# Yelp/nrtsearch

Hardware: AMD Instinct MI355X
Metric: queries/sec, 10M-doc 5-term BM25 top-1000 (higher is better)
Workload: dtype f32

## Files before the change

nrtsearch_amd/csrc/maxscore.hip:

```cpp
#include <hip/hip_runtime.h>
#include <stdint.h>

#include <type_traits>

#include "bm25_common.hiph"

namespace nrtgpu {

constexpr int kMsWinWords = kMsWinDocs / 32;
constexpr int kSl = kMsSlots;
typedef uint32_t u32x2 __attribute__((ext_vector_type(2)));
typedef const NRT_GLOBAL u32x2* gvec2_ptr;

struct alignas(16) WClause {
  uint64_t docids, fnorm;
  uint64_t begin;
  uint32_t count, pad0;
  float    weight;
  int32_t  fx_scale;
  uint32_t flags;
  uint32_t pad;
  uint64_t u_after;
  uint64_t look;
  uint64_t cells, start;
};
static_assert(sizeof(WClause) == 80, "WClause layout");

struct MsSmem {
  uint64_t cand[kMsCandCap];
  uint32_t tab[kTabTerms][kTabEntries];
  float    cache[kLdsCaches][256];
  uint32_t seen[kMsWaves][kMsWinWords];
  WClause  wc[kMsWaves][kMsMaxTerms];
  TopkScratch sc;
  uint64_t theta;
  uint64_t thr;
  uint32_t cnt;
  uint32_t cnt_valid;
  uint32_t rz_flag;
  uint32_t spec_busy;
  uint32_t spec_meet;
  uint32_t n_meet, n_over, n_est;
  uint32_t wins_started;
  uint32_t spec_at;
  uint32_t q_wins;
  uint32_t spec_z16;
  uint32_t spec_grow16;
  unsigned long long* spec_slot;
  uint64_t pick;
  uint32_t role[4];
  uint32_t prune_on;
  uint32_t slot_hits[kSliceSlots];
  uint32_t slot_slice[kSliceSlots];
  uint64_t prof[16];
};
static_assert(sizeof(MsSmem) <= 160 * 1024, "the MaxScore workgroup owns one CU's 160 KiB LDS");

__device__ __forceinline__ uint64_t uniform_u64(uint64_t v) {
  const uint32_t lo = (uint32_t)__builtin_amdgcn_readfirstlane((int)(uint32_t)v);
  const uint32_t hi = (uint32_t)__builtin_amdgcn_readfirstlane((int)(uint32_t)(v >> 32));
  return ((uint64_t)hi << 32) | (uint64_t)lo;
}
__device__ __forceinline__ uint64_t readlane_u64(uint64_t v, uint32_t l) {
  const uint32_t lo = (uint32_t)__builtin_amdgcn_readlane((int)(uint32_t)v, (int)l);
  const uint32_t hi = (uint32_t)__builtin_amdgcn_readlane((int)(uint32_t)(v >> 32), (int)l);
  return ((uint64_t)hi << 32) | (uint64_t)lo;
}

template <bool PACKED, int NS>
__device__ __forceinline__ void values_of_codes(const MsSmem& s, const uint32_t (&c)[NS], uint32_t need, uint32_t tab_slot,
                                                float w, int fx_scale, uint32_t cache_slot, uint64_t esc_list,
                                                const uint32_t (&pidx)[NS], uint32_t (&val)[NS]) {
  const uint32_t tab = tab_slot < (uint32_t)kTabTerms ? tab_slot : 7u;
  const char* tb = (const char*)&s.tab[tab == 7u ? 0u : tab][0];
  uint32_t cor = 0;
#pragma unroll
  for (int j = 0; j < NS; ++j) {
    val[j] = *(const uint32_t*)(tb + (c[j] & 0x1FFCu));
    const uint32_t cn = ((need >> j) & 1u) ? c[j] : 0u;
    cor = PACKED ? max(cor, cn) : (cor | cn);
  }
  const bool special = need != 0u && ((PACKED ? cor >= (kPackEscBase << 2) : (cor >> 31) != 0u) || tab == 7u);
  if (__any(special)) {
    const float* cache = &s.cache[cache_slot][0];
#pragma unroll
    for (int j = 0; j < NS; ++j) {
      uint32_t cj = c[j];
      if (PACKED && cj >= (kPackEscBase << 2)) cj = ((need >> j) & 1u) ? packed_escape_word((gu32_ptr)esc_list, pidx[j], cj >> 2) : 0x80000100u;
      const bool esc = (cj >> 31) != 0u;
      const uint32_t f = esc ? ((cj >> 8) & 0x3FFFFFu) : ((cj >> 9) & 15u);
      const bool dead = esc ? ((cj >> 30) & 1u) != 0u : (cj >> 20) != 0u;
      const uint32_t nb = esc ? (cj & 255u) : ((cj >> 2) & 127u);
      if (((need >> j) & 1u) && (esc || tab == 7u))
        val[j] = dead ? 0u : score_value<true>(bm25_score(w, (float)(int32_t)f, cache[nb]), fx_scale);
    }
  }
}

#ifdef NRT_MS_PHASE_CLOCKS
#define NRT_PH_MARK(i)                                                          \
  do {                                                                          \
    if (PROF) {                                                                 \
      asm volatile("s_waitcnt vmcnt(0) lgkmcnt(0)" ::: "memory");               \
      const uint64_t t_ph_ = __builtin_readcyclecounter();                      \
      ph[i] += t_ph_ - ph_t;                                                    \
      ph_t = t_ph_;                                                             \
    }                                                                           \
  } while (0)
#else
#define NRT_PH_MARK(i) do {} while (0)
#endif
typedef const __attribute__((address_space(4))) MsArgs* ms_args_ptr;
template <class T>
__device__ __forceinline__ T* as_global(T* p) { return (T*)(NRT_GLOBAL T*)p; }
__device__ __forceinline__ ms_args_ptr ms_fresh(const MsArgs* p) {
  uint32_t lo = (uint32_t)(uintptr_t)p, hi = (uint32_t)((uintptr_t)p >> 32);
  asm volatile("" : "+v"(lo), "+v"(hi));
  lo = (uint32_t)__builtin_amdgcn_readfirstlane((int)lo);
  hi = (uint32_t)__builtin_amdgcn_readfirstlane((int)hi);
  return (ms_args_ptr)(((uintptr_t)hi << 32) | (uintptr_t)lo);
}

__device__ __noinline__ void ms_compact(__attribute__((address_space(3))) MsSmem* sp, uint32_t k, int fx_E,
                                        unsigned long long* theta_g, const DExchange* xch, uint32_t query) {
  MsSmem& s = *(MsSmem*)sp;
  const uint32_t tid = threadIdx.x;
  const uint32_t cnt_raw = s.cnt;
  const uint32_t cnt0 = cnt_raw > (uint32_t)kMsCandCap ? s.cnt_valid : cnt_raw;
#ifdef NRTGPU_DEV
  const bool keep_live = (s.spec_meet & 4u) == 0u;
#else
  constexpr bool keep_live = true;
#endif
  const uint64_t tg_in = tid == 0 && keep_live ? (uint64_t)__hip_atomic_load(theta_g, __ATOMIC_RELAXED, __HIP_MEMORY_SCOPE_AGENT) : 0ull;
  __syncthreads();
  if (tid == 0) {
    s.n_meet += 1u;
    if (cnt_raw > (uint32_t)kMsCandCap) s.n_over += 1u;
    if (tg_in > s.theta) {
      s.theta = tg_in;
      s.thr = acc_threshold<true>(tg_in, fx_E);
    }
  }
  const bool exchanging = xch && xch->world > 1u;
  uint32_t r = 0;
  if (s.spec_z16 != 0u && !exchanging && __hip_atomic_load(&s.prune_on, __ATOMIC_RELAXED, __HIP_MEMORY_SCOPE_WORKGROUP) != 0u) {
    const float m = (float)k * fminf(1.0f, (float)s.wins_started / (float)max(s.q_wins, 1u));
    const float rr = m + (float)s.spec_z16 * (1.0f / 16.0f) * sqrtf(m) + 2.0f;
    r = rr < (float)k ? (uint32_t)rr : 0u;
  }
  uint64_t guess = 0;
  if (cnt0 > k) {
    const uint32_t k2 = exchanging ? (k + xch->world - 2u) / (xch->world - 1u) : r;
    const uint64_t thr = topk_kth_union<kMsThreads>(s.cand, cnt0, k, &s.sc, [](auto&&) {}, k2);
    const uint32_t q2_hi = s.sc.q2_hi;
    uint64_t keep = thr;
    if (keep_live) {
      const uint64_t edge = !exchanging && r != 0u && q2_hi != 0u ? (uint64_t)q2_hi << 32 : 0ull, th_in = s.theta;
      if (edge > keep) keep = edge;
      if (th_in > keep) keep = th_in;
    }
    const uint32_t kept = topk_keep_ge<kMsThreads, kMsCandCap>(s.cand, cnt0, keep, &s.sc);
    for (uint32_t i = kept + tid; i < (uint32_t)kMsCandCap; i += kMsThreads) s.cand[i] = 0ull;
    if (tid == 0) {
      s.cnt = kept;
      if (thr > s.theta) {
        s.theta = thr;
        s.thr = acc_threshold<true>(thr, fx_E);
      }
      atomicMax(theta_g, (unsigned long long)thr);
      s.prof[1] += 1;
    }
    if (!exchanging && r != 0u && q2_hi != 0u) guess = (uint64_t)q2_hi << 32;
    if (xch && tid < 64u) {
      const uint64_t pb = exchange_bound(*xch, query, q2_hi != 0u ? (uint64_t)q2_hi << 32 : 0ull, tid);
      if (tid == 0 && pb > s.theta) {
        s.theta = pb;
        s.thr = acc_threshold<true>(pb, fx_E);
        atomicMax(theta_g, (unsigned long long)pb);
      }
    }
  } else {
    if (r != 0u && cnt0 > r) guess = topk_kth_union<kMsThreads>(s.cand, cnt0, r, &s.sc, [](auto&&) {}, 0u);
    if (tid == 0) s.cnt = cnt0;
  }
  if (tid == 0 && s.spec_z16 != 0u) {
    if (guess > s.theta) {
      s.theta = guess;
      s.thr = acc_threshold<true>(guess, fx_E);
      atomicMax(theta_g, (unsigned long long)guess);
      atomicMax(s.spec_slot, (unsigned long long)guess);
      s.n_est += 0x10000u;
    }
    const uint32_t ws = s.wins_started;
    s.spec_at = ws >= s.q_wins ? 0u : max(ws * s.spec_grow16 / 16u, ws + (uint32_t)kMsWaves);
  }
  __syncthreads();
  if (tid == 0) s.rz_flag = 0;
  __syncthreads();
}

__device__ __forceinline__ bool ms_meet(MsSmem& s, uint32_t k, int fx_E, unsigned long long* theta_g, const DExchange* xch = nullptr,
                                        uint32_t query = 0) {
  __syncthreads();
  if (!__hip_atomic_load(&s.rz_flag, __ATOMIC_RELAXED, __HIP_MEMORY_SCOPE_WORKGROUP)) return false;
  ms_compact((__attribute__((address_space(3))) MsSmem*)&s, k, fx_E, theta_g, xch, query);
  return true;
}

__device__ __noinline__ void ms_estimate(__attribute__((address_space(3))) MsSmem* sp, uint32_t k, int fx_E,
                                         unsigned long long* theta_g, const DExchange* xch) {
  MsSmem& s = *(MsSmem*)sp;
  const uint32_t lane = threadIdx.x & 63u;
  const uint32_t ws = (uint32_t)__builtin_amdgcn_readfirstlane((int)__hip_atomic_load(&s.wins_started, __ATOMIC_RELAXED, __HIP_MEMORY_SCOPE_WORKGROUP));
  const uint32_t at = (uint32_t)__builtin_amdgcn_readfirstlane((int)__hip_atomic_load(&s.spec_at, __ATOMIC_RELAXED, __HIP_MEMORY_SCOPE_WORKGROUP));
  const uint32_t n = (uint32_t)__builtin_amdgcn_readfirstlane((int)__hip_atomic_load(&s.cnt, __ATOMIC_RELAXED, __HIP_MEMORY_SCOPE_WORKGROUP));
  if (at != 0u && ws >= at && n <= (uint32_t)kMsCandCap) {
    const bool exchanging = xch && xch->world > 1u;
    uint32_t r = 0;
    if (s.spec_z16 != 0u && !exchanging && __hip_atomic_load(&s.prune_on, __ATOMIC_RELAXED, __HIP_MEMORY_SCOPE_WORKGROUP) != 0u) {
      const float m = (float)k * fminf(1.0f, (float)ws / (float)max(s.q_wins, 1u));
      const float rr = m + (float)s.spec_z16 * (1.0f / 16.0f) * sqrtf(m) + 2.0f;
      r = rr < (float)k ? (uint32_t)rr : 0u;
    }
    uint64_t guess = 0;
    if (r != 0u && n > r) guess = topk_kth_wave(s.cand, n, r, &s.sc);
    if (lane == 0u) {
      if (guess > s.theta) {
        __hip_atomic_store(&s.theta, guess, __ATOMIC_RELAXED, __HIP_MEMORY_SCOPE_WORKGROUP);
        __hip_atomic_store(&s.thr, acc_threshold<true>(guess, fx_E), __ATOMIC_RELAXED, __HIP_MEMORY_SCOPE_WORKGROUP);
        atomicMax(theta_g, (unsigned long long)guess);
        atomicMax(s.spec_slot, (unsigned long long)guess);
      }
      s.spec_at = ws >= s.q_wins ? 0u : max(ws * s.spec_grow16 / 16u, ws + (uint32_t)kMsWaves);
      s.n_est += 1u;
    }
  }
  wave_lds_phase();
  if (lane == 0u) __hip_atomic_store(&s.spec_busy, 0u, __ATOMIC_RELEASE, __HIP_MEMORY_SCOPE_WORKGROUP);
}

__device__ __forceinline__ bool ms_reserve(MsSmem& s, uint32_t lane, uint32_t mine, uint32_t& pos) {
  const uint32_t incl = scan64_dpp(mine);
  const uint32_t wave_total = (uint32_t)__builtin_amdgcn_readlane((int)incl, 63);
  uint32_t wbase = 0;
  if (lane == 0) {
    wbase = atomicAdd(&s.cnt, wave_total);
    if (wbase + wave_total > (uint32_t)kMsCandCap) {
      if (wbase <= (uint32_t)kMsCandCap) s.cnt_valid = wbase;
      __hip_atomic_store(&s.rz_flag, 1u, __ATOMIC_RELAXED, __HIP_MEMORY_SCOPE_WORKGROUP);
    }
  }
  wbase = (uint32_t)__builtin_amdgcn_readfirstlane((int)wbase);
  pos = wbase + incl - mine;
  return wbase + wave_total <= (uint32_t)kMsCandCap;
}

template <bool PROF, bool PACKED, int SHAPES>
__global__ __launch_bounds__(kMsThreads)
void bm25_maxscore_kernel(const MsArgs* __restrict__ launch) {
  constexpr bool TWO = SHAPES == 2;
  constexpr bool kMsHalfBody = kSl == 8;
  __shared__ MsSmem s;
  const uint32_t tid = threadIdx.x;
  const uint32_t wave = tid >> 6, lane = tid & 63u;
  for (uint32_t round = 0;; ++round) {
    const uint64_t wall_entry = PROF ? wall_clock64() : 0ull;
    const ms_args_ptr ap = ms_fresh(launch);
    const __attribute__((address_space(4))) DHelp& hp = ap->help;
    const DItem* const items = as_global(ap->items);
    const DPart* const parts = as_global(ap->parts);
    const DWalkRow* const rows = as_global(ap->rows);
  #ifdef NRTGPU_DEV
    const DTerm* const terms = as_global(ap->terms);
  #endif
    const DExchange* const xch = as_global(ap->xch);
    bool helper = false;
    uint32_t my_item = 0, out_slot = 0;
    {
      const uint32_t min_rem = hp.min_rem & 0xFFFFu;
      const bool greedy = ((hp.min_rem >> 16) & 1u) != 0u;
      for (int attempt = 0; attempt < 2; ++attempt) {
        if (tid == 0) {
          s.pick = 0ull;
          s.role[0] = __hip_atomic_load(hp.item_next, __ATOMIC_RELAXED, __HIP_MEMORY_SCOPE_AGENT);
          s.role[1] = __hip_atomic_load(hp.help_used, __ATOMIC_RELAXED, __HIP_MEMORY_SCOPE_AGENT);
          s.role[2] = 0u;
          s.role[3] = __hip_atomic_load(hp.help_off, __ATOMIC_RELAXED, __HIP_MEMORY_SCOPE_AGENT);
        }
        __syncthreads();
        const uint32_t q_next = s.role[0];
        const bool queue_empty = attempt == 1 || q_next >= hp.n_own;
        const bool slots_left = s.role[1] < hp.n_help;
        if (queue_empty && (!slots_left || s.role[3] != 0u)) return;
        const bool look = slots_left && (queue_empty || (hp.alpha16 != 0u && q_next >= hp.n_cus + hp.n_cus / 4u));
        if (look) {
          const uint64_t now = wall_clock64();
          float t_rem = 0.f;
          if (!queue_empty) {
            uint32_t mine = 0;
            for (uint32_t i = tid; i < hp.n_own; i += kMsThreads) {
              const uint64_t t0 = __hip_atomic_load(hp.item_t0 + i, __ATOMIC_RELAXED, __HIP_MEMORY_SCOPE_AGENT);
              if (t0 == 0ull) continue;
              mine += min(items[i].flags >> 8, (uint32_t)kMsWaves + __hip_atomic_load(hp.win_next + i, __ATOMIC_RELAXED, __HIP_MEMORY_SCOPE_AGENT));
            }
            mine = (uint32_t)__builtin_amdgcn_readlane((int)scan64_dpp(mine), 63);
            if (lane == 0 && mine != 0u) atomicAdd(&s.role[2], mine);
            __syncthreads();
            const uint32_t handed = s.role[2];
            const uint64_t ts = __hip_atomic_load(hp.t_start, __ATOMIC_RELAXED, __HIP_MEMORY_SCOPE_AGENT);
            t_rem = (handed == 0u || ts == 0ull || now <= ts) ? 3.0e38f
                    : (float)(now - ts) * (float)(hp.total_wins > handed ? hp.total_wins - handed : 0u) / (float)handed * ((float)hp.alpha16 * (1.0f / 16.0f));
          }
          for (uint32_t i = tid; i < hp.n_own; i += kMsThreads) {
            const uint32_t fl = items[i].flags;
            if ((fl & 3u) == kMsModeExact) continue;
            const uint32_t nw = fl >> 8;
            const uint32_t taken = (uint32_t)kMsWaves + __hip_atomic_load(hp.win_next + i, __ATOMIC_RELAXED, __HIP_MEMORY_SCOPE_AGENT);
            if (taken + min_rem > nw) continue;
            const uint64_t t0 = __hip_atomic_load(hp.item_t0 + i, __ATOMIC_RELAXED, __HIP_MEMORY_SCOPE_AGENT);
            if (t0 == 0ull || now <= t0) continue;
            const uint32_t hc = __hip_atomic_load(hp.help_cnt + i, __ATOMIC_RELAXED, __HIP_MEMORY_SCOPE_AGENT);
            const float left = (float)(now - t0) * (float)(nw - taken) / ((float)(taken - (uint32_t)kMsWaves + 1u) * (float)(1u + hc));
            if (!queue_empty && !(left > t_rem)) continue;
            uint32_t hsh = ((blockIdx.x + round * gridDim.x) * 0x9E3779B9u) ^ (i * 0x85EBCA6Bu) ^ (uint32_t)now;
            hsh ^= hsh >> 16; hsh *= 0x7FEB352Du; hsh ^= hsh >> 15; hsh *= 0x846CA68Bu; hsh ^= hsh >> 16;
            const float u = ((float)(hsh >> 8) + 0.5f) * (1.0f / 16777216.0f);
            const float key = greedy ? left : left / -__logf(u);
            atomicMax((unsigned long long*)&s.pick, ((unsigned long long)__float_as_uint(key) << 32) | (unsigned long long)(i + 1u));
          }
        }
        __syncthreads();
        if (tid == 0) {
          const uint64_t pick = s.pick;
          uint32_t r_item = 0xFFFFFFFFu, r_slot = 0xFFFFFFFFu;
          if ((uint32_t)pick != 0u) {
            const uint32_t slot = atomicAdd(hp.help_used, 1u);
            if (slot < hp.n_help) {
              r_slot = slot;
              r_item = (uint32_t)pick - 1u;
              atomicAdd(hp.help_cnt + r_item, 1u);
            }
          } else if (queue_empty && look) {
            __hip_atomic_store(hp.help_off, 1u, __ATOMIC_RELAXED, __HIP_MEMORY_SCOPE_AGENT);
          }
          if (r_slot == 0xFFFFFFFFu && !queue_empty) {
            const uint32_t it = atomicAdd(hp.item_next, 1u);
            if (it < hp.n_own) r_item = it;
          }
          s.role[0] = r_item;
          s.role[1] = r_slot;
        }
        __syncthreads();
        const uint32_t r_item = s.role[0], r_slot = s.role[1];
        __syncthreads();
        if (r_item != 0xFFFFFFFFu) {
          my_item = r_item;
          helper = r_slot != 0xFFFFFFFFu;
          out_slot = helper ? hp.slot_base + r_slot : r_item;
          break;
        }
        if (queue_empty) return;
      }
    }
    NRT_GLOBAL uint32_t* const win_next_g = (NRT_GLOBAL uint32_t*)(hp.win_next + my_item);
    uint32_t first_win = 0;
    if (helper && lane == 0) first_win = __hip_atomic_fetch_add(win_next_g, 1u, __ATOMIC_RELAXED, __HIP_MEMORY_SCOPE_AGENT);
    const DItem item = items[my_item];
    const DQuery q = as_global(ap->queries)[item.query];
    const uint32_t k = q.k;
    const int fx_E = item.fx_E;
    unsigned long long* const my_theta_g = as_global(ap->theta_g) + item.query;
    const bool multi_item = q.n_items > 1 || hp.n_help != 0u;
    const uint32_t mode = item.flags & 3u;
    const uint32_t win_tiles = (uint32_t)kMsWinTiles >> ((item.flags >> 2) & 3u);
    const uint32_t msm = SHAPES ? q.min_should_match : 0u;
    const bool use_max = SHAPES && q.combine_max != 0u;
    const uint32_t sec_mode = TWO ? q.sec_mode : kMsSecNone;
    const float tie_breaker = TWO ? q.tie_breaker : 0.0f;
    auto loosen = [&](uint64_t t) { return (TWO && sec_mode == kMsSecReqOpt) ? max(t - (t >> 21), (uint64_t)2) - (uint64_t)1 : t; };
    unsigned int* const my_prune_g = as_global(ap->q_prune) + item.query;
    const uint64_t after_key = q.has_after ? pack_key(q.after_score, (uint32_t)q.after_doc) : ~0ull;

    {
      const uint32_t n_lds = min(item.n_caches, (uint32_t)kLdsCaches) * 256u;
      const float* const caches = as_global(ap->caches);
      for (uint32_t i = tid; i < n_lds; i += kMsThreads) (&s.cache[0][0])[i] = caches[item.cache_off + i];
    }
    for (uint32_t i = tid; i < (uint32_t)kMsCandCap; i += kMsThreads) s.cand[i] = 0ull;
    if (tid == 0) {
      const uint64_t theta0 = __hip_atomic_load(my_theta_g, __ATOMIC_RELAXED, __HIP_MEMORY_SCOPE_AGENT);
      s.theta = theta0;
      s.thr = acc_threshold<true>(theta0, fx_E);
      s.cnt = 0;
      s.cnt_valid = 0;
      s.rz_flag = 0;
      s.spec_busy = 0;
      s.n_meet = s.n_over = s.n_est = 0;
      if (!helper) {
        const unsigned long long now0 = (unsigned long long)wall_clock64();
        __hip_atomic_store(hp.item_t0 + my_item, now0, __ATOMIC_RELAXED, __HIP_MEMORY_SCOPE_AGENT);
        if (my_item == 0u) __hip_atomic_store(hp.t_start, now0, __ATOMIC_RELAXED, __HIP_MEMORY_SCOPE_AGENT);
      }
      s.prune_on = mode == kMsModePrune ? 1u : 0u;
      const bool spec = hp.spec_g != nullptr && hp.spec_z16 != 0u;
      s.wins_started = 0;
      s.q_wins = spec ? as_global(ap->q_wins)[item.query] : 0u;
      s.spec_z16 = spec ? hp.spec_z16 : 0u;
      s.spec_slot = spec ? as_global(hp.spec_g) + item.query : nullptr;
      s.spec_at = spec ? max(hp.spec_sched & 255u, 1u) : 0u;
      s.spec_grow16 = max((hp.spec_sched >> 8) & 255u, 17u);
      s.spec_meet = (hp.spec_sched >> 16) & 7u;
      for (int i = 0; i < kSliceSlots; ++i) s.slot_hits[i] = s.slot_slice[i] = 0u;
      for (int i = 0; i < 16; ++i) s.prof[i] = 0;
    }
    const uint64_t t_item0 = PROF ? __builtin_readcyclecounter() : 0ull;
    const uint64_t wall0 = PROF ? wall_clock64() : 0ull;
    uint64_t tc_meet = 0, tc_part = 0, tc_walk = 0;
    __syncthreads();
    if (xch && tid < 64u) {
      const uint64_t pb = exchange_bound(*xch, item.query, 0ull, tid);
      if (tid == 0 && pb > s.theta) {
        s.theta = pb;
        s.thr = acc_threshold<true>(pb, fx_E);
      }
    }
    for (uint32_t slot = 0; slot < item.n_tabs; ++slot) {
      const float w = items[my_item].tab_weight[slot];
      const int scale = items[my_item].tab_scale[slot];
      const float* cache = &s.cache[items[my_item].tab_cache[slot]][0];
      for (uint32_t e = tid; e < (uint32_t)kTabEntries; e += kMsThreads)
        s.tab[slot][e] = e < (uint32_t)kTabNorms ? 0u : score_value<true>(bm25_score(w, (float)(int32_t)(e >> 7), cache[e & 127u]), scale);
    }
    __syncthreads();
  #if !defined(NRT_MS_PHASE_CLOCKS) && !defined(NRT_MS_COUNT_ROUNDS)
    if (PROF && tid == 0) s.prof[8] = __builtin_readcyclecounter() - t_item0;
  #endif

    uint32_t* const seen = &s.seen[wave][0];
    WClause* const wcl = &s.wc[wave][0];
    const uint32_t wcl_addr = lds_addr(wcl);
    uint32_t wave_hits = 0;
    uint32_t cur_slot = 0;
    uint64_t pc_post = 0, pc_surv = 0, pc_look = 0, pc_cand = 0, pc_chunks = 0, pc_wins = 0;
  #ifdef NRT_MS_PHASE_CLOCKS
    uint64_t ph[9] = {0, 0, 0, 0, 0, 0, 0, 0, 0}, ph_t = 0;
  #endif
  #ifdef NRT_MS_COUNT_ROUNDS
    uint64_t pc_dense = 0, pc_sparse = 0, pc_steps = 0, pc_tas = 0, pc_crounds = 0, pc_half = 0, pc_half_rounds = 0;
    uint64_t pc_cres = 0, pc_cinst = 0;
  #endif
    const uint32_t item_wins = item.flags >> 8;
    uint32_t sc_mul = 1u;
    if (ap->scatter != 0u && item_wins > 3u && item_wins < 65536u) {
      const uint32_t primes[4] = {2654435761u, 2246822519u, 3266489917u, 668265263u};
      uint32_t best = 0xFFFFFFFFu;
  #pragma unroll
      for (int i = 0; i < 4; ++i) {
        const uint32_t a = primes[i] % item_wins;
        const uint32_t x = a * 1000u, y = item_wins * 618u;
        const uint32_t dist = x > y ? x - y : y - x;
        if (a > 1u && dist < best) {
          best = dist;
          sc_mul = a;
        }
      }
    }
    auto window_of_take = [&](uint32_t h) -> uint32_t {
      return (sc_mul == 1u || h >= item_wins) ? h : (h * sc_mul) % item_wins;
    };
    uint32_t g = window_of_take(helper ? (uint32_t)kMsWaves + (uint32_t)__builtin_amdgcn_readfirstlane((int)first_win) : wave);
    uint32_t pi = 0;
    uint32_t win_base = 0;

    const bool parts_by_lane = item.n_parts <= 64u;
    uint32_t part_incl = 0;
    if (parts_by_lane) {
      uint32_t w = 0;
      if (lane < item.n_parts) {
        const u32x2 tr = *(gvec2_ptr)&parts[item.part_begin + lane].tile_begin;
        w = (tr[1] - (tr[0] & ~(win_tiles - 1u)) + win_tiles - 1u) / win_tiles;
      }
      part_incl = scan64_dpp(w);
    }

    for (;;) {
      DPart part;
      uint32_t part_wins = 0;
      if (parts_by_lane) {
        const uint64_t holds = __builtin_amdgcn_ballot_w64(lane < item.n_parts && g < part_incl);
        if (holds == 0ull) break;
        pi = (uint32_t)__builtin_ctzll(holds);
        part = parts[item.part_begin + pi];
        part_wins = (part.tile_end - (part.tile_begin & ~(win_tiles - 1u)) + win_tiles - 1u) / win_tiles;
        win_base = (uint32_t)__builtin_amdgcn_readlane((int)part_incl, (int)pi) - part_wins;
      } else {
        if (sc_mul != 1u) {
          pi = 0;
          win_base = 0;
        }
        for (;; ++pi) {
          if (pi >= item.n_parts) break;
          part = parts[item.part_begin + pi];
          part_wins = (part.tile_end - (part.tile_begin & ~(win_tiles - 1u)) + win_tiles - 1u) / win_tiles;
          if (g < win_base + part_wins) break;
          win_base += part_wins;
        }
      }
      if (pi >= item.n_parts) break;
      {
        const uint32_t p_slot = part.slice >> 24;
        if (p_slot != cur_slot && wave_hits != 0u) {
          if (lane == 0) atomicAdd(&s.slot_hits[cur_slot], wave_hits);
          wave_hits = 0;
// ... 501 lines not shown
            else if (TWO && sec_mode == kMsSecReqOpt)
              score = acc_score<true>(rsel - ssel, fx_E) + acc_score<true>(ssel, fx_E);
            const uint64_t key = pack_key(score, (uint32_t)(part.doc_base + (int32_t)dsel));
            const bool want = low != 0u && key > theta_now && key < after_key;
            uint32_t pos = 0;
            if (!__any(want)) {
              maybe &= ~low;
              continue;
            }
  #ifdef NRT_MS_COUNT_ROUNDS
            if (PROF) pc_cres += 1;
  #endif
            if (ms_reserve(s, lane, want ? 1u : 0u, pos)) {
              if (want) s.cand[pos] = key;
              if (PROF) pc_cand += want ? 1u : 0u;
              maybe &= ~low;
              continue;
            }
            const uint64_t t_m0 = PROF ? __builtin_readcyclecounter() : 0ull;
            (void)ms_meet(s, k, fx_E, my_theta_g, xch, item.query);
            if (PROF) tc_meet += __builtin_readcyclecounter() - t_m0;
            theta_now = max(theta_now, s.theta);
          }
  #ifdef NRT_MS_COUNT_ROUNDS
          if (PROF && pc_cres != cres0) pc_cinst += 1;
  #endif
          }
          NRT_PH_MARK(8);
          return true;
        };
        for (uint32_t v0 = 0; v0 < n_groups; v0 += 64u) {
          bool more;
          if (kMsHalfBody && n_groups - v0 <= 32u && half_on) {
  #ifdef NRT_MS_COUNT_ROUNDS
            const uint64_t chunks0 = pc_chunks, look0 = pc_dense + pc_sparse;
  #endif
            if constexpr (kMsHalfBody) more = walk_units(std::integral_constant<int, 4>{}, std::true_type{}, v0);
            else more = false;
  #ifdef NRT_MS_COUNT_ROUNDS
            if (PROF) {
              pc_half += pc_chunks - chunks0;
              pc_half_rounds += pc_dense + pc_sparse - look0;
            }
  #endif
          } else {
            more = walk_units(std::integral_constant<int, kSl>{}, std::false_type{}, v0);
          }
          if (!more) break;
          if (__hip_atomic_load(&s.rz_flag, __ATOMIC_RELAXED, __HIP_MEMORY_SCOPE_WORKGROUP)) {
            const uint64_t t_m0 = PROF ? __builtin_readcyclecounter() : 0ull;
            (void)ms_meet(s, k, fx_E, my_theta_g, xch, item.query);
            if (PROF) tc_meet += __builtin_readcyclecounter() - t_m0;
          }
        }

        if (PROF) tc_walk += __builtin_readcyclecounter() - t_win0;
        g = window_of_take((uint32_t)__builtin_amdgcn_readfirstlane((int)g_new));
        if (g < win_base || g >= win_base + part_wins) break;
      }
    }
    const uint64_t t_idle0 = PROF ? __builtin_readcyclecounter() : 0ull;
    while (ms_meet(s, k, fx_E, my_theta_g, xch, item.query)) {
    }
    const uint64_t t_epi0 = PROF ? __builtin_readcyclecounter() : 0ull;
    if (PROF && lane == 0) {
      atomicAdd((unsigned long long*)&s.prof[10], (unsigned long long)tc_meet);
      atomicAdd((unsigned long long*)&s.prof[11], (unsigned long long)(t_epi0 - t_idle0));
      atomicAdd((unsigned long long*)&s.prof[12], (unsigned long long)tc_part);
      atomicAdd((unsigned long long*)&s.prof[13], (unsigned long long)(tc_walk - tc_meet));
  #ifndef NRT_MS_COUNT_ROUNDS
      atomicMax((unsigned long long*)&s.prof[14], (unsigned long long)(t_idle0 - t_item0));
  #else
      atomicAdd((unsigned long long*)&s.prof[14], (unsigned long long)pc_half | ((unsigned long long)pc_half_rounds << 32));
      atomicAdd((unsigned long long*)&s.prof[11], (unsigned long long)pc_tas - (unsigned long long)(t_epi0 - t_idle0));
      atomicAdd((unsigned long long*)&s.prof[12], (unsigned long long)pc_dense - (unsigned long long)tc_part);
      atomicAdd((unsigned long long*)&s.prof[10], (unsigned long long)pc_sparse - (unsigned long long)tc_meet);
      atomicAdd((unsigned long long*)&s.prof[13], (unsigned long long)pc_steps - (unsigned long long)(tc_walk - tc_meet));
      atomicAdd((unsigned long long*)&s.prof[8], (unsigned long long)pc_crounds);
      atomicAdd((unsigned long long*)&s.prof[9], (unsigned long long)pc_cres);
      atomicAdd((unsigned long long*)&s.prof[15], (unsigned long long)pc_cinst);
  #endif
    }

    {
      const uint32_t c = s.cnt;
      __syncthreads();
      if (c > k) {
        uint64_t thr = 0;
        const uint32_t m = topk_compact<kMsThreads, kMsCandCap>(s.cand, c, k, &s.sc, &thr);
        if (tid == 0) s.cnt = m;
      }
    }
    if (lane == 0 && wave_hits) atomicAdd(&s.slot_hits[cur_slot], wave_hits);
  #ifdef NRT_MS_PHASE_CLOCKS
    if (PROF && lane == 0) {
  #pragma unroll
      for (int i = 0; i < 9; ++i) atomicAdd((unsigned long long*)&s.prof[i], (unsigned long long)ph[i]);
    }
    if (false) {
  #else
    if (PROF && lane == 0) {
      atomicAdd((unsigned long long*)&s.prof[0], (unsigned long long)pc_wins);
      atomicAdd((unsigned long long*)&s.prof[2], (unsigned long long)pc_chunks);
    }
    if (PROF) {
  #endif
      uint64_t v3 = pc_post, v4 = pc_surv, v6 = pc_look, v7 = pc_cand;
  #pragma unroll
      for (int dlt = 32; dlt > 0; dlt >>= 1) {
        v3 += __shfl_xor(v3, dlt, 64);
        v4 += __shfl_xor(v4, dlt, 64);
        v6 += __shfl_xor(v6, dlt, 64);
        v7 += __shfl_xor(v7, dlt, 64);
      }
      if (lane == 0) {
        atomicAdd((unsigned long long*)&s.prof[3], (unsigned long long)v3);
        atomicAdd((unsigned long long*)&s.prof[4], (unsigned long long)v4);
        atomicAdd((unsigned long long*)&s.prof[6], (unsigned long long)v6);
        atomicAdd((unsigned long long*)&s.prof[7], (unsigned long long)v7);
      }
    }
    __syncthreads();
    const uint32_t n_held = s.cnt;
    const ms_args_ptr ape = ms_fresh(launch);
    const __attribute__((address_space(4))) DHelp& hpe = ape->help;
    uint64_t* out = as_global(ape->item_keys) + (size_t)out_slot * ape->k_stride;
    if (tid == 0) {
      uint64_t th_end = s.theta;
      if (multi_item) {
        const uint64_t tg = (uint64_t)__hip_atomic_load(my_theta_g, __ATOMIC_RELAXED, __HIP_MEMORY_SCOPE_AGENT);
        if (tg > th_end) th_end = tg;
      }
      s.thr = th_end;
      s.cnt_valid = 0u;
    }
    __syncthreads();
    for (uint32_t i = tid; i < n_held; i += kMsThreads) {
      const uint64_t key = s.cand[i];
      if (key >= s.thr) out[atomicAdd(&s.cnt_valid, 1u)] = key;
    }
    __syncthreads();
    const uint32_t n = s.cnt_valid;
    if (tid == 0) {
      as_global(ape->item_counts)[out_slot] = n;
      if (helper)
        as_global(hpe.help_query)[out_slot - hpe.slot_base] = item.query + 1u;
      uint32_t hits = 0;
      for (int i = 0; i < kSliceSlots; ++i) {
        const uint32_t h = s.slot_hits[i];
        hits += h;
        if (h != 0u && q.gte_floor != 0xFFFFFFFFu) atomicAdd(as_global(ape->slice_sum) + q.slice_base + s.slot_slice[i], h);
      }
      const bool pruned = s.prune_on != 0u && (s.theta != 0ull || __hip_atomic_load(my_theta_g, __ATOMIC_RELAXED, __HIP_MEMORY_SCOPE_AGENT) != 0ull);
      as_global(ape->item_hits)[out_slot] = (uint64_t)hits + (pruned ? kHitsPrunedUnit : 0ull);
      if (PROF && ape->item_prof) {
  #ifndef NRT_MS_PHASE_CLOCKS
        s.prof[5] = hits;
        s.prof[1] = (s.prof[1] & 0xFFFull) | ((uint64_t)min(s.n_meet, 0xFFFu) << 12) | ((uint64_t)min(s.n_over, 0xFFFu) << 24) |
                    ((uint64_t)min(s.n_est & 0xFFFFu, 0xFFFu) << 36) | ((uint64_t)min(s.n_est >> 16, 0xFFFu) << 48);
  #endif
  #ifndef NRT_MS_COUNT_ROUNDS
        const uint64_t t_end = __builtin_readcyclecounter();
        s.prof[9] = t_end - t_item0;
        s.prof[15] = t_end - t_epi0;
  #endif
        for (int i = 0; i < 16; ++i) as_global(ape->item_prof)[(size_t)out_slot * 16 + i] = s.prof[i];
        if (hpe.walls) {
          unsigned long long* const wr = as_global(hpe.walls) + (size_t)out_slot * 8;
          wr[0] = wall0;
          wr[1] = wall_clock64();
          wr[2] = (unsigned long long)my_item | ((unsigned long long)item.flags << 32);
          wr[3] = s.prof[0];
          wr[4] = wall_entry;
          wr[5] = ((unsigned long long)((uint32_t)__builtin_amdgcn_s_getreg((31 << 11) | 20) & 15u) << 8) |
                  (unsigned long long)(((uint32_t)__builtin_amdgcn_s_getreg((31 << 11) | 4) >> 8) & 255u);
          wr[6] = (unsigned long long)round | ((unsigned long long)item.query << 32);
          wr[7] = blockIdx.x;
        }
      }
    }
    if (hpe.persistent == 0u) return;
    __syncthreads();
  }
}

__global__ __launch_bounds__(256)
void term_frontier_kernel(const uint32_t* __restrict__ fnorm, const uint64_t* __restrict__ t_start,
                          const uint32_t* __restrict__ t_count, const uint64_t* __restrict__ t_look,
                          const uint32_t* __restrict__ t_meta, const char* __restrict__ look_base, DTermAux* __restrict__ out) {
  __shared__ uint32_t mn[13];
  __shared__ uint32_t mf;
  const uint32_t t = blockIdx.x;
  if (threadIdx.x < 13) mn[threadIdx.x] = 0xFFu;
  if (threadIdx.x == 13) mf = 0u;
  __syncthreads();
  const uint64_t st = t_start[t];
  const uint32_t n = t_count[t];
  uint32_t lmn[13];
  uint32_t lmf = 0;
#pragma unroll
  for (int i = 0; i < 13; ++i) lmn[i] = 0xFFu;
  for (uint32_t p = threadIdx.x; p < n; p += 256u) {
    const uint32_t c = fnorm[st + p];
    if (c >> 31) {
      lmn[12] = min(lmn[12], c & 255u);
      lmf = max(lmf, (c >> 8) & 0x3FFFFFu);
    } else {
      const uint32_t f = (c >> 9) & 15u, nb = (c >> 2) & 127u;
#pragma unroll
      for (int i = 0; i < 12; ++i)
        if (f == (uint32_t)(i + 1)) lmn[i] = min(lmn[i], nb);
    }
  }
#pragma unroll
  for (int i = 0; i < 13; ++i)
    if (lmn[i] != 0xFFu) atomicMin(&mn[i], lmn[i]);
  if (lmf) atomicMax(&mf, lmf);
  __syncthreads();
  if (threadIdx.x == 0) {
    DTermAux a;
    const bool has = t_look[t] != ~0ull;
    a.look = has ? (const void*)(look_base + t_look[t]) : nullptr;
    for (int i = 0; i < 12; ++i) a.min_norm[i] = (uint8_t)mn[i];
    a.esc_min_norm = (uint8_t)mn[12];
    a.look_kind = has ? (uint8_t)(t_meta[t] & 255u) : (uint8_t)kLookNone;
    a.look_shift = has ? (uint8_t)((t_meta[t] >> 8) & 255u) : (uint8_t)0;
    a.pad = 0;
    a.esc_max_freq = mf;
    a.pad2 = 0;
    out[t] = a;
  }
}

__global__ __launch_bounds__(256)
void term_bits_kernel(const uint32_t* __restrict__ docids, const uint64_t* __restrict__ t_start, const uint32_t* __restrict__ t_count,
                      const uint64_t* __restrict__ t_look, const uint32_t* __restrict__ which, char* __restrict__ look_base) {
  const uint32_t t = which[blockIdx.y];
  const uint64_t st = t_start[t];
  const uint32_t n = t_count[t];
  uint32_t* const r = (uint32_t*)(look_base + t_look[t]);
  const uint32_t stride = gridDim.x * blockDim.x;
  for (uint32_t p = blockIdx.x * blockDim.x + threadIdx.x; p < n; p += stride) {
    const uint32_t d = docids[st + p];
    const uint32_t blk = d >> 5;
    atomicOr(&r[(size_t)blk * 2u], 1u << (d & 31u));
    if (p == 0u || (docids[st + p - 1u] >> 5) != blk) r[(size_t)blk * 2u + 1u] = p;
  }
}

__global__ __launch_bounds__(256)
void term_cells_kernel(const uint32_t* __restrict__ docids, const uint64_t* __restrict__ t_start, const uint32_t* __restrict__ t_count,
                       const uint64_t* __restrict__ t_look, const uint32_t* __restrict__ t_meta, const uint32_t* __restrict__ which,
                       uint32_t max_doc, char* __restrict__ look_base) {
  const uint32_t t = which[blockIdx.y];
  const uint32_t* const dd = docids + t_start[t];
  const uint32_t n = t_count[t];
  const uint32_t shift = (t_meta[t] >> 8) & 255u;
  const uint32_t n_cells = ((max_doc - 1u) >> shift) + 1u;
  uint32_t* const out = (uint32_t*)(look_base + t_look[t]);
  const uint32_t stride = gridDim.x * blockDim.x;
  for (uint32_t i = blockIdx.x * blockDim.x + threadIdx.x; i <= n_cells; i += stride) {
    const uint64_t bound = (uint64_t)i << shift;
    uint32_t lo = 0, hi = n;
    while (lo < hi) {
      const uint32_t mid = (lo + hi) >> 1;
// ... 80 lines not shown
```

Baseline: 570,900.

## Outline scheduler and epilogue, parallelize per-item prologue and output compaction

Moves the work-item selection loop into a noinline ms_choose that prefetches the per-item state once and reuses it for both the handed sum and the draw, and moves the top-k compaction and output write into a noinline ms_finish. The output write now uses a wave ballot with one LDS atomic per wave instead of one per key, and the slice-hit sums use a shuffle reduction instead of a serial loop on thread 0. Per-item prologue values (tab weights, scales, cache ids, theta, q_wins) are loaded into LDS by spare threads rather than re-read from global memory in the table build. Kernarg pointer reloads now go through kernarg_segment_ptr. The aim is lower per-item fixed overhead and register pressure in the persistent kernel, at the cost of extra function-call and synchronisation overhead plus more complex role handoff through LDS.

```diff
diff --git a/nrtsearch_amd/csrc/maxscore.hip b/nrtsearch_amd/csrc/maxscore.hip
--- a/nrtsearch_amd/csrc/maxscore.hip
+++ b/nrtsearch_amd/csrc/maxscore.hip
@@ -26,6 +26,13 @@
 };
 static_assert(sizeof(WClause) == 80, "WClause layout");
 
+struct MsTurn {
+  uint64_t pick;
+  uint64_t t_start;
+  uint32_t q_next, used, off;
+  uint32_t handed;
+  uint32_t r_item, pad;
+};
 struct MsSmem {
   uint64_t cand[kMsCandCap];
   uint32_t tab[kTabTerms][kTabEntries];
@@ -47,11 +54,17 @@
   uint32_t spec_z16;
   uint32_t spec_grow16;
   unsigned long long* spec_slot;
-  uint64_t pick;
-  uint32_t role[4];
+  MsTurn   turn[2];
   uint32_t prune_on;
   uint32_t slot_hits[kSliceSlots];
   uint32_t slot_slice[kSliceSlots];
+  float    tab_weight[kTabTerms];
+  uint32_t tab_cache[kTabTerms];
+  int32_t  tab_scale[kTabTerms];
+  uint64_t choice;
+  uint32_t fin_slot;
+  uint32_t fin_flags;
+  uint32_t fin_floor, fin_slice;
   uint64_t prof[16];
 };
 static_assert(sizeof(MsSmem) <= 160 * 1024, "the MaxScore workgroup owns one CU's 160 KiB LDS");
@@ -114,11 +127,15 @@
 template <class T>
 __device__ __forceinline__ T* as_global(T* p) { return (T*)(NRT_GLOBAL T*)p; }
 __device__ __forceinline__ ms_args_ptr ms_fresh(const MsArgs* p) {
-  uint32_t lo = (uint32_t)(uintptr_t)p, hi = (uint32_t)((uintptr_t)p >> 32);
-  asm volatile("" : "+v"(lo), "+v"(hi));
-  lo = (uint32_t)__builtin_amdgcn_readfirstlane((int)lo);
-  hi = (uint32_t)__builtin_amdgcn_readfirstlane((int)hi);
-  return (ms_args_ptr)(((uintptr_t)hi << 32) | (uintptr_t)lo);
+  (void)p;
+  uintptr_t ka = (uintptr_t)__builtin_amdgcn_kernarg_segment_ptr();
+  asm volatile("" : "+s"(ka));
+  return *(const ms_args_ptr __attribute__((address_space(4)))*)ka;
+}
+
+__device__ __forceinline__ uint32_t ms_here(uint32_t v) {
+  asm volatile("" : "+v"(v));
+  return v;
 }
 
 __device__ __noinline__ void ms_compact(__attribute__((address_space(3))) MsSmem* sp, uint32_t k, int fx_E,
@@ -256,6 +273,186 @@
   return wbase + wave_total <= (uint32_t)kMsCandCap;
 }
 
+constexpr int kChooseItems = 2;
+constexpr uint64_t kChoiceNone = ~0ull;
+__device__ __noinline__ void ms_choose(__attribute__((address_space(3))) MsSmem* sp, ms_args_ptr ap, uint32_t round) {
+  MsSmem& s = *(MsSmem*)sp;
+  const __attribute__((address_space(4))) DHelp& hp = ap->help;
+  const DItem* const items = as_global(ap->items);
+  const uint32_t tid = threadIdx.x, lane = tid & 63u;
+  const uint32_t n_own = hp.n_own, n_help = hp.n_help;
+  const uint32_t min_rem = hp.min_rem & 0xFFFFu;
+  const bool greedy = ((hp.min_rem >> 16) & 1u) != 0u;
+  const unsigned long long* const item_t0 = as_global(hp.item_t0);
+  const uint32_t* const win_next = as_global(hp.win_next);
+  const uint32_t* const help_cnt = as_global(hp.help_cnt);
+  struct Look { uint64_t t0; uint32_t wn, hc, fl; };
+  auto look_at = [&](uint32_t i, Look& l) {
+    l.t0 = __hip_atomic_load(item_t0 + i, __ATOMIC_RELAXED, __HIP_MEMORY_SCOPE_AGENT);
+    l.wn = __hip_atomic_load(win_next + i, __ATOMIC_RELAXED, __HIP_MEMORY_SCOPE_AGENT);
+    l.hc = __hip_atomic_load(help_cnt + i, __ATOMIC_RELAXED, __HIP_MEMORY_SCOPE_AGENT);
+    l.fl = items[i].flags;
+  };
+  auto handed_of = [&](const Look& l) -> uint32_t { return l.t0 == 0ull ? 0u : min(l.fl >> 8, (uint32_t)kMsWaves + l.wn); };
+  for (uint32_t attempt = 0; attempt < 2u; ++attempt) {
+    MsTurn& t = s.turn[attempt];
+    const uint64_t now = wall_clock64();
+    uint32_t e_next = 0, e_used = 0, e_off = 0;
+    uint64_t e_ts = 0;
+    if (tid == 0) {
+      e_next = __hip_atomic_load(hp.item_next, __ATOMIC_RELAXED, __HIP_MEMORY_SCOPE_AGENT);
+      e_used = __hip_atomic_load(hp.help_used, __ATOMIC_RELAXED, __HIP_MEMORY_SCOPE_AGENT);
+      e_off = __hip_atomic_load(hp.help_off, __ATOMIC_RELAXED, __HIP_MEMORY_SCOPE_AGENT);
+      e_ts = __hip_atomic_load(hp.t_start, __ATOMIC_RELAXED, __HIP_MEMORY_SCOPE_AGENT);
+    }
+    Look mine[kChooseItems] = {};
+#pragma unroll
+    for (int j = 0; j < kChooseItems; ++j) {
+      const uint32_t i = tid + (uint32_t)j * (uint32_t)kMsThreads;
+      if (i < n_own) look_at(i, mine[j]);
+    }
+    uint32_t sum = 0;
+#pragma unroll
+    for (int j = 0; j < kChooseItems; ++j) sum += handed_of(mine[j]);
+    for (uint32_t i = tid + (uint32_t)(kChooseItems * kMsThreads); i < n_own; i += kMsThreads) {
+      Look l;
+      look_at(i, l);
+      sum += handed_of(l);
+    }
+    sum = (uint32_t)__builtin_amdgcn_readlane((int)scan64_dpp(sum), 63);
+    if (lane == 0 && sum != 0u) atomicAdd(&t.handed, sum);
+    if (tid == 0) {
+      t.q_next = e_next;
+      t.used = e_used;
+      t.off = e_off;
+      t.t_start = e_ts;
+    }
+    __syncthreads();
+    const uint32_t q_next = t.q_next;
+    const bool queue_empty = attempt == 1u || q_next >= n_own;
+    const bool slots_left = t.used < n_help;
+    if (queue_empty && (!slots_left || t.off != 0u)) {
+      s.choice = kChoiceNone;
+      return;
+    }
+    const bool look = slots_left && (queue_empty || (hp.alpha16 != 0u && q_next >= hp.n_cus + hp.n_cus / 4u));
+    if (look) {
+      float t_rem = 0.f;
+      if (!queue_empty) {
+        const uint32_t handed = t.handed;
+        const uint64_t ts = t.t_start;
+        t_rem = (handed == 0u || ts == 0ull || now <= ts) ? 3.0e38f
+                : (float)(now - ts) * (float)(hp.total_wins > handed ? hp.total_wins - handed : 0u) / (float)handed * ((float)hp.alpha16 * (1.0f / 16.0f));
+      }
+      auto draw = [&](uint32_t i, const Look& l) {
+        if ((l.fl & 3u) == kMsModeExact) return;
+        const uint32_t nw = l.fl >> 8;
+        const uint32_t taken = (uint32_t)kMsWaves + l.wn;
+        if (taken + min_rem > nw) return;
+        if (l.t0 == 0ull || now <= l.t0) return;
+        const float left = (float)(now - l.t0) * (float)(nw - taken) / ((float)(taken - (uint32_t)kMsWaves + 1u) * (float)(1u + l.hc));
+        if (!queue_empty && !(left > t_rem)) return;
+        uint32_t hsh = ((blockIdx.x + round * gridDim.x) * 0x9E3779B9u) ^ (i * 0x85EBCA6Bu) ^ (uint32_t)now;
+        hsh ^= hsh >> 16; hsh *= 0x7FEB352Du; hsh ^= hsh >> 15; hsh *= 0x846CA68Bu; hsh ^= hsh >> 16;
+        const float u = ((float)(hsh >> 8) + 0.5f) * (1.0f / 16777216.0f);
+        const float key = greedy ? left : left / -__logf(u);
+        atomicMax((unsigned long long*)&t.pick, ((unsigned long long)__float_as_uint(key) << 32) | (unsigned long long)(i + 1u));
+      };
+#pragma unroll
+      for (int j = 0; j < kChooseItems; ++j) {
+        const uint32_t i = tid + (uint32_t)j * (uint32_t)kMsThreads;
+        if (i < n_own) draw(i, mine[j]);
+      }
+      for (uint32_t i = tid + (uint32_t)(kChooseItems * kMsThreads); i < n_own; i += kMsThreads) {
+        Look l;
+        look_at(i, l);
+        draw(i, l);
+      }
+    }
+    __syncthreads();
+    if (tid == 0) {
+      const uint64_t pick = t.pick;
+      uint32_t r_item = 0xFFFFFFFFu, r_slot = 0xFFFFFFFFu;
+      if ((uint32_t)pick != 0u) {
+        const uint32_t slot = atomicAdd(hp.help_used, 1u);
+        if (slot < n_help) {
+          r_slot = slot;
+          r_item = (uint32_t)pick - 1u;
+          atomicAdd(hp.help_cnt + r_item, 1u);
+        }
+      } else if (queue_empty && look) {
+        __hip_atomic_store(hp.help_off, 1u, __ATOMIC_RELAXED, __HIP_MEMORY_SCOPE_AGENT);
+      }
+      if (r_slot == 0xFFFFFFFFu && !queue_empty) {
+        const uint32_t it = atomicAdd(hp.item_next, 1u);
+        if (it < n_own) r_item = it;
+      }
+      t.r_item = r_item;
+      s.choice = r_item != 0xFFFFFFFFu ? ((uint64_t)r_slot << 32) | (uint64_t)r_item : kChoiceNone;
+    }
+    __syncthreads();
+    if (t.r_item != 0xFFFFFFFFu || queue_empty) return;
+  }
+}
+
+__device__ __noinline__ uint32_t ms_finish(__attribute__((address_space(3))) MsSmem* sp, ms_args_ptr ap, uint32_t k, unsigned long long* theta_g,
+                                           uint32_t query) {
+  MsSmem& s = *(MsSmem*)sp;
+  const uint32_t tid = threadIdx.x, lane = tid & 63u;
+  const uint32_t flags = s.fin_flags, out_slot = s.fin_slot, gte_floor = s.fin_floor, slice_base = s.fin_slice;
+  const __attribute__((address_space(4))) DHelp& hp = ap->help;
+  uint64_t tg_end = 0;
+  if (tid == 0) tg_end = (uint64_t)__hip_atomic_load(theta_g, __ATOMIC_RELAXED, __HIP_MEMORY_SCOPE_AGENT);
+  {
+    const uint32_t c = s.cnt;
+    __syncthreads();
+    if (c > k) {
+      uint64_t thr = 0;
+      const uint32_t m = topk_compact<kMsThreads, kMsCandCap>(s.cand, c, k, &s.sc, &thr);
+      if (tid == 0) s.cnt = m;
+    }
+  }
+  if (tid == 0) {
+    uint64_t th_end = s.theta;
+    if ((flags & 2u) != 0u && tg_end > th_end) th_end = tg_end;
+    s.thr = th_end;
+    s.cnt_valid = 0u;
+  }
+  __syncthreads();
+  const uint32_t n_held = s.cnt;
+  const uint64_t th_out = s.thr;
+  uint64_t* out = as_global(ap->item_keys) + (size_t)out_slot * ap->k_stride;
+  for (uint32_t i = tid; (i & ~63u) < n_held; i += kMsThreads) {
+    const uint64_t key = i < n_held ? s.cand[i] : 0ull;
+    const bool keep = i < n_held && key >= th_out;
+    const uint64_t keepers = __builtin_amdgcn_ballot_w64(keep);
+    if (keepers != 0ull) {
+      uint32_t base = 0;
+      if (lane == 0) base = atomicAdd(&s.cnt_valid, (uint32_t)__builtin_popcountll(keepers));
+      base = (uint32_t)__builtin_amdgcn_readfirstlane((int)base);
+      if (keep) out[base + __builtin_amdgcn_mbcnt_hi((uint32_t)(keepers >> 32), __builtin_amdgcn_mbcnt_lo((uint32_t)keepers, 0u))] = key;
+    }
+  }
+  __syncthreads();
+  const uint32_t n = s.cnt_valid;
+  uint32_t hits = 0;
+  if (tid < 64u) {
+    const uint32_t h = tid < (uint32_t)kSliceSlots ? s.slot_hits[tid] : 0u;
+    if (h != 0u && gte_floor != 0xFFFFFFFFu) atomicAdd(as_global(ap->slice_sum) + slice_base + s.slot_slice[tid], h);
+    hits = h;
+#pragma unroll
+    for (int dlt = kSliceSlots / 2; dlt > 0; dlt >>= 1) hits += (uint32_t)__shfl_xor((int)hits, dlt, 64);
+  }
+  if (tid == 0) {
+    as_global(ap->item_counts)[out_slot] = n;
+    if ((flags & 1u) != 0u)
+      as_global(hp.help_query)[out_slot - hp.slot_base] = query + 1u;
+    const bool pruned = s.prune_on != 0u && (s.theta != 0ull || tg_end != 0ull);
+    as_global(ap->item_hits)[out_slot] = (uint64_t)hits + (pruned ? kHitsPrunedUnit : 0ull);
+  }
+  return hits;
+}
+
 template <bool PROF, bool PACKED, int SHAPES>
 __global__ __launch_bounds__(kMsThreads)
 void bm25_maxscore_kernel(const MsArgs* __restrict__ launch) {
@@ -264,8 +461,16 @@
   __shared__ MsSmem s;
   const uint32_t tid = threadIdx.x;
   const uint32_t wave = tid >> 6, lane = tid & 63u;
+  if (tid == 0) {
+    s.turn[0].pick = s.turn[1].pick = 0ull;
+    s.turn[0].handed = s.turn[1].handed = 0u;
+  }
+  __syncthreads();
   for (uint32_t round = 0;; ++round) {
     const uint64_t wall_entry = PROF ? wall_clock64() : 0ull;
+    ms_choose((__attribute__((address_space(3))) MsSmem*)&s, ms_fresh(launch), round);
+    const uint64_t choice = s.choice;
+    if (choice == kChoiceNone) return;
     const ms_args_ptr ap = ms_fresh(launch);
     const __attribute__((address_space(4))) DHelp& hp = ap->help;
     const DItem* const items = as_global(ap->items);
@@ -275,94 +480,9 @@
     const DTerm* const terms = as_global(ap->terms);
   #endif
     const DExchange* const xch = as_global(ap->xch);
-    bool helper = false;
-    uint32_t my_item = 0, out_slot = 0;
-    {
-      const uint32_t min_rem = hp.min_rem & 0xFFFFu;
-      const bool greedy = ((hp.min_rem >> 16) & 1u) != 0u;
-      for (int attempt = 0; attempt < 2; ++attempt) {
-        if (tid == 0) {
-          s.pick = 0ull;
-          s.role[0] = __hip_atomic_load(hp.item_next, __ATOMIC_RELAXED, __HIP_MEMORY_SCOPE_AGENT);
-          s.role[1] = __hip_atomic_load(hp.help_used, __ATOMIC_RELAXED, __HIP_MEMORY_SCOPE_AGENT);
-          s.role[2] = 0u;
-          s.role[3] = __hip_atomic_load(hp.help_off, __ATOMIC_RELAXED, __HIP_MEMORY_SCOPE_AGENT);
-        }
-        __syncthreads();
-        const uint32_t q_next = s.role[0];
-        const bool queue_empty = attempt == 1 || q_next >= hp.n_own;
-        const bool slots_left = s.role[1] < hp.n_help;
-        if (queue_empty && (!slots_left || s.role[3] != 0u)) return;
-        const bool look = slots_left && (queue_empty || (hp.alpha16 != 0u && q_next >= hp.n_cus + hp.n_cus / 4u));
-        if (look) {
-          const uint64_t now = wall_clock64();
-          float t_rem = 0.f;
-          if (!queue_empty) {
-            uint32_t mine = 0;
-            for (uint32_t i = tid; i < hp.n_own; i += kMsThreads) {
-              const uint64_t t0 = __hip_atomic_load(hp.item_t0 + i, __ATOMIC_RELAXED, __HIP_MEMORY_SCOPE_AGENT);
-              if (t0 == 0ull) continue;
-              mine += min(items[i].flags >> 8, (uint32_t)kMsWaves + __hip_atomic_load(hp.win_next + i, __ATOMIC_RELAXED, __HIP_MEMORY_SCOPE_AGENT));
-            }
-            mine = (uint32_t)__builtin_amdgcn_readlane((int)scan64_dpp(mine), 63);
-            if (lane == 0 && mine != 0u) atomicAdd(&s.role[2], mine);
-            __syncthreads();
-            const uint32_t handed = s.role[2];
-            const uint64_t ts = __hip_atomic_load(hp.t_start, __ATOMIC_RELAXED, __HIP_MEMORY_SCOPE_AGENT);
-            t_rem = (handed == 0u || ts == 0ull || now <= ts) ? 3.0e38f
-                    : (float)(now - ts) * (float)(hp.total_wins > handed ? hp.total_wins - handed : 0u) / (float)handed * ((float)hp.alpha16 * (1.0f / 16.0f));
-          }
-          for (uint32_t i = tid; i < hp.n_own; i += kMsThreads) {
-            const uint32_t fl = items[i].flags;
-            if ((fl & 3u) == kMsModeExact) continue;
-            const uint32_t nw = fl >> 8;
-            const uint32_t taken = (uint32_t)kMsWaves + __hip_atomic_load(hp.win_next + i, __ATOMIC_RELAXED, __HIP_MEMORY_SCOPE_AGENT);
-            if (taken + min_rem > nw) continue;
-            const uint64_t t0 = __hip_atomic_load(hp.item_t0 + i, __ATOMIC_RELAXED, __HIP_MEMORY_SCOPE_AGENT);
-            if (t0 == 0ull || now <= t0) continue;
-            const uint32_t hc = __hip_atomic_load(hp.help_cnt + i, __ATOMIC_RELAXED, __HIP_MEMORY_SCOPE_AGENT);
-            const float left = (float)(now - t0) * (float)(nw - taken) / ((float)(taken - (uint32_t)kMsWaves + 1u) * (float)(1u + hc));
-            if (!queue_empty && !(left > t_rem)) continue;
-            uint32_t hsh = ((blockIdx.x + round * gridDim.x) * 0x9E3779B9u) ^ (i * 0x85EBCA6Bu) ^ (uint32_t)now;
-            hsh ^= hsh >> 16; hsh *= 0x7FEB352Du; hsh ^= hsh >> 15; hsh *= 0x846CA68Bu; hsh ^= hsh >> 16;
-            const float u = ((float)(hsh >> 8) + 0.5f) * (1.0f / 16777216.0f);
-            const float key = greedy ? left : left / -__logf(u);
-            atomicMax((unsigned long long*)&s.pick, ((unsigned long long)__float_as_uint(key) << 32) | (unsigned long long)(i + 1u));
-          }
-        }
-        __syncthreads();
-        if (tid == 0) {
-          const uint64_t pick = s.pick;
-          uint32_t r_item = 0xFFFFFFFFu, r_slot = 0xFFFFFFFFu;
-          if ((uint32_t)pick != 0u) {
-            const uint32_t slot = atomicAdd(hp.help_used, 1u);
-            if (slot < hp.n_help) {
-              r_slot = slot;
-              r_item = (uint32_t)pick - 1u;
-              atomicAdd(hp.help_cnt + r_item, 1u);
-            }
-          } else if (queue_empty && look) {
-            __hip_atomic_store(hp.help_off, 1u, __ATOMIC_RELAXED, __HIP_MEMORY_SCOPE_AGENT);
-          }
-          if (r_slot == 0xFFFFFFFFu && !queue_empty) {
-            const uint32_t it = atomicAdd(hp.item_next, 1u);
-            if (it < hp.n_own) r_item = it;
-          }
-          s.role[0] = r_item;
-          s.role[1] = r_slot;
-        }
-        __syncthreads();
-        const uint32_t r_item = s.role[0], r_slot = s.role[1];
-        __syncthreads();
-        if (r_item != 0xFFFFFFFFu) {
-          my_item = r_item;
-          helper = r_slot != 0xFFFFFFFFu;
-          out_slot = helper ? hp.slot_base + r_slot : r_item;
-          break;
-        }
-        if (queue_empty) return;
-      }
-    }
+    const uint32_t my_item = (uint32_t)choice;
+    const bool helper = (uint32_t)(choice >> 32) != 0xFFFFFFFFu;
+    const uint32_t out_slot = helper ? hp.slot_base + (uint32_t)(choice >> 32) : my_item;
     NRT_GLOBAL uint32_t* const win_next_g = (NRT_GLOBAL uint32_t*)(hp.win_next + my_item);
     uint32_t first_win = 0;
     if (helper && lane == 0) first_win = __hip_atomic_fetch_add(win_next_g, 1u, __ATOMIC_RELAXED, __HIP_MEMORY_SCOPE_AGENT);
@@ -382,14 +502,48 @@
     unsigned int* const my_prune_g = as_global(ap->q_prune) + item.query;
     const uint64_t after_key = q.has_after ? pack_key(q.after_score, (uint32_t)q.after_doc) : ~0ull;
 
+    const bool spec = hp.spec_g != nullptr && hp.spec_z16 != 0u;
+    uint64_t theta0 = 0;
+    uint32_t q_wins0 = 0;
+    if (tid == 0) {
+      theta0 = __hip_atomic_load(my_theta_g, __ATOMIC_RELAXED, __HIP_MEMORY_SCOPE_AGENT);
+      if (spec) q_wins0 = as_global(ap->q_wins)[item.query];
+    }
+    const uint32_t tabs_n = min(item.n_tabs, (uint32_t)kTabTerms);
+    float tab_w = 0.f;
+    uint32_t tab_c = 0;
+    int tab_s = 0;
+    const uint32_t tid_p = ms_here(tid);
+    const uint32_t z_pro = (uint32_t)kMsThreads - 1u - tid_p;
+    if (z_pro < tabs_n) {
+      const uint32_t z = z_pro;
+      tab_w = items[my_item].tab_weight[z];
+      tab_c = items[my_item].tab_cache[z];
+      tab_s = items[my_item].tab_scale[z];
+    }
     {
       const uint32_t n_lds = min(item.n_caches, (uint32_t)kLdsCaches) * 256u;
       const float* const caches = as_global(ap->caches);
-      for (uint32_t i = tid; i < n_lds; i += kMsThreads) (&s.cache[0][0])[i] = caches[item.cache_off + i];
-    }
-    for (uint32_t i = tid; i < (uint32_t)kMsCandCap; i += kMsThreads) s.cand[i] = 0ull;
+      for (uint32_t i = tid_p; i < n_lds; i += kMsThreads) (&s.cache[0][0])[i] = caches[item.cache_off + i];
+    }
+    for (uint32_t i = tid_p; i < (uint32_t)kMsCandCap; i += kMsThreads) s.cand[i] = 0ull;
+    {
+      const uint32_t z = z_pro;
+      if (z < (uint32_t)kSliceSlots) s.slot_hits[z] = s.slot_slice[z] = 0u;
+      if (z < 16u) s.prof[z] = 0;
+      if (z < tabs_n) {
+        s.tab_weight[z] = tab_w;
+        s.tab_cache[z] = tab_c;
+        s.tab_scale[z] = tab_s;
+      }
+    }
     if (tid == 0) {
-      const uint64_t theta0 = __hip_atomic_load(my_theta_g, __ATOMIC_RELAXED, __HIP_MEMORY_SCOPE_AGENT);
+      s.turn[0].pick = s.turn[1].pick = 0ull;
+      s.turn[0].handed = s.turn[1].handed = 0u;
+      s.fin_slot = out_slot;
+      s.fin_flags = (helper ? 1u : 0u) | (multi_item ? 2u : 0u);
+      s.fin_floor = q.gte_floor;
+      s.fin_slice = q.slice_base;
       s.theta = theta0;
       s.thr = acc_threshold<true>(theta0, fx_E);
       s.cnt = 0;
@@ -403,16 +557,13 @@
         if (my_item == 0u) __hip_atomic_store(hp.t_start, now0, __ATOMIC_RELAXED, __HIP_MEMORY_SCOPE_AGENT);
       }
       s.prune_on = mode == kMsModePrune ? 1u : 0u;
-      const bool spec = hp.spec_g != nullptr && hp.spec_z16 != 0u;
       s.wins_started = 0;
-      s.q_wins = spec ? as_global(ap->q_wins)[item.query] : 0u;
+      s.q_wins = q_wins0;
       s.spec_z16 = spec ? hp.spec_z16 : 0u;
       s.spec_slot = spec ? as_global(hp.spec_g) + item.query : nullptr;
       s.spec_at = spec ? max(hp.spec_sched & 255u, 1u) : 0u;
       s.spec_grow16 = max((hp.spec_sched >> 8) & 255u, 17u);
       s.spec_meet = (hp.spec_sched >> 16) & 7u;
-      for (int i = 0; i < kSliceSlots; ++i) s.slot_hits[i] = s.slot_slice[i] = 0u;
-      for (int i = 0; i < 16; ++i) s.prof[i] = 0;
     }
     const uint64_t t_item0 = PROF ? __builtin_readcyclecounter() : 0ull;
     const uint64_t wall0 = PROF ? wall_clock64() : 0ull;
@@ -426,10 +577,10 @@
       }
     }
     for (uint32_t slot = 0; slot < item.n_tabs; ++slot) {
-      const float w = items[my_item].tab_weight[slot];
-      const int scale = items[my_item].tab_scale[slot];
-      const float* cache = &s.cache[items[my_item].tab_cache[slot]][0];
-      for (uint32_t e = tid; e < (uint32_t)kTabEntries; e += kMsThreads)
+      const float w = s.tab_weight[slot];
+      const int scale = s.tab_scale[slot];
+      const float* cache = &s.cache[s.tab_cache[slot]][0];
+      for (uint32_t e = tid_p; e < (uint32_t)kTabEntries; e += kMsThreads)
         s.tab[slot][e] = e < (uint32_t)kTabNorms ? 0u : score_value<true>(bm25_score(w, (float)(int32_t)(e >> 7), cache[e & 127u]), scale);
     }
     __syncthreads();
@@ -1097,15 +1248,6 @@
   #endif
     }
 
-    {
-      const uint32_t c = s.cnt;
-      __syncthreads();
-      if (c > k) {
-        uint64_t thr = 0;
-        const uint32_t m = topk_compact<kMsThreads, kMsCandCap>(s.cand, c, k, &s.sc, &thr);
-        if (tid == 0) s.cnt = m;
-      }
-    }
     if (lane == 0 && wave_hits) atomicAdd(&s.slot_hits[cur_slot], wave_hits);
   #ifdef NRT_MS_PHASE_CLOCKS
     if (PROF && lane == 0) {
@@ -1135,40 +1277,12 @@
         atomicAdd((unsigned long long*)&s.prof[7], (unsigned long long)v7);
       }
     }
-    __syncthreads();
-    const uint32_t n_held = s.cnt;
+    const uint32_t hits = ms_finish((__attribute__((address_space(3))) MsSmem*)&s, ms_fresh(launch), k, my_theta_g, item.query);
     const ms_args_ptr ape = ms_fresh(launch);
     const __attribute__((address_space(4))) DHelp& hpe = ape->help;
-    uint64_t* out = as_global(ape->item_keys) + (size_t)out_slot * ape->k_stride;
-    if (tid == 0) {
-      uint64_t th_end = s.theta;
-      if (multi_item) {
-        const uint64_t tg = (uint64_t)__hip_atomic_load(my_theta_g, __ATOMIC_RELAXED, __HIP_MEMORY_SCOPE_AGENT);
-        if (tg > th_end) th_end = tg;
-      }
-      s.thr = th_end;
-      s.cnt_valid = 0u;
-    }
-    __syncthreads();
-    for (uint32_t i = tid; i < n_held; i += kMsThreads) {
-      const uint64_t key = s.cand[i];
-      if (key >= s.thr) out[atomicAdd(&s.cnt_valid, 1u)] = key;
-    }
-    __syncthreads();
-    const uint32_t n = s.cnt_valid;
-    if (tid == 0) {
-      as_global(ape->item_counts)[out_slot] = n;
-      if (helper)
-        as_global(hpe.help_query)[out_slot - hpe.slot_base] = item.query + 1u;
-      uint32_t hits = 0;
-      for (int i = 0; i < kSliceSlots; ++i) {
-        const uint32_t h = s.slot_hits[i];
-        hits += h;
-        if (h != 0u && q.gte_floor != 0xFFFFFFFFu) atomicAdd(as_global(ape->slice_sum) + q.slice_base + s.slot_slice[i], h);
-      }
-      const bool pruned = s.prune_on != 0u && (s.theta != 0ull || __hip_atomic_load(my_theta_g, __ATOMIC_RELAXED, __HIP_MEMORY_SCOPE_AGENT) != 0ull);
-      as_global(ape->item_hits)[out_slot] = (uint64_t)hits + (pruned ? kHitsPrunedUnit : 0ull);
-      if (PROF && ape->item_prof) {
+    if (PROF && tid == 0 && ape->item_prof) {
+      {
+        const uint32_t out_slot = s.fin_slot;
   #ifndef NRT_MS_PHASE_CLOCKS
         s.prof[5] = hits;
         s.prof[1] = (s.prof[1] & 0xFFFull) | ((uint64_t)min(s.n_meet, 0xFFFu) << 12) | ((uint64_t)min(s.n_over, 0xFFFu) << 24) |
@@ -1195,7 +1309,6 @@
       }
     }
     if (hpe.persistent == 0u) return;
-    __syncthreads();
   }
 }
 
```

New measurement: 574,900 (median of 6 runs). No clear change (+0.7%).
